# JoshuaLim007/VoxelEngine

Measured on AMD Instinct MI355X. Metric: Mrays/s primary+1-bounce @1080p, 8k×512×8k brickmap; % HBM roofline, higher is better.
Workload: dtype f32

## Files before the change

voxelengine_amd/csrc/vxrt_api.hip:

```cpp
#include "../../include/vxrt.h"
#include "vxrt_dist.hpp"
#include "vxrt_edit.hpp"
#include "vxrt_kernels.hpp"
#include "vxrt_islands.hpp"
#include "vxrt_nav.hpp"
#include "vxrt_region.hpp"
#include "vxrt_stream.hpp"

#include <algorithm>
#include <atomic>
#include <cmath>
#include <cstdio>
#include <cstdlib>
#include <cstring>
#include <initializer_list>
#include <map>
#include <new>
#include <set>
#include <string>
#include <utility>
#include <vector>

namespace vxrt {
hipError_t launch_render(const RenderArgs& A, bool stats, int variant, hipStream_t stream);
// ... 822 lines not shown
    VX_HIP(hipSetDevice(c->device));
    VX_HIP(hipDeviceSynchronize());
    unsigned long long now[vxrt::kStatCount] = {}, h[vxrt::kStatCount];
    std::vector<unsigned long long> rows((size_t)vxrt::kStatRows * vxrt::kStatRowStride);
    VX_HIP(hipMemcpy(rows.data(), c->d_stats, rows.size() * sizeof(unsigned long long), hipMemcpyDeviceToHost));
    for (unsigned r = 0; r < vxrt::kStatRows; ++r)
        for (int i = 0; i < vxrt::kStatCount; ++i)
            now[i] += rows[(size_t)r * vxrt::kStatRowStride + i];
    for (int i = 0; i < vxrt::kStatCount; ++i) {
        h[i] = now[i] - c->stats_base[i];
        c->stats_base[i] = now[i];
    }
    out->primary_rays = h[vxrt::kStatPrimary];
    out->shadow_rays = h[vxrt::kStatShadow];
    out->bounce_rays = h[vxrt::kStatBounce];
    out->primary_hits = h[vxrt::kStatPrimaryHits];
    out->coarse_probes = h[vxrt::kStatCoarseProbes];
    out->brick_entries = h[vxrt::kStatBrickEntries];
    out->fine_probes = h[vxrt::kStatFineProbes];
    out->dbg[0] = h[vxrt::kStatDbgIters];
    out->dbg[1] = h[vxrt::kStatDbgWalkLanes];
    out->dbg[2] = h[vxrt::kStatDbgEndRuns];
    out->dbg[3] = h[vxrt::kStatDbgBoxRuns];
    out->dbg[4] = h[vxrt::kStatDbgNextRuns];
    out->dbg[5] = h[vxrt::kStatDbgEndLanes];
    out->dbg[6] = h[vxrt::kStatDbgBoxLanes];
    out->dbg[7] = h[vxrt::kStatDbgNextLanes];
    out->dbg[8] = h[vxrt::kStatDbgLifetime];
    out->dbg[9] = h[vxrt::kStatDbgDrained];
    out->dbg[10] = h[vxrt::kStatDbgNextTicks];
    out->dbg[11] = h[vxrt::kStatDbgParkTicks];
    out->guard_slack_loads = h[vxrt::kStatGuardSlack];
    out->guard_stray_loads = h[vxrt::kStatGuardStray];
    return VXRT_OK;
}

int vxrt_deinterleave_strips(vxrt_ctx* c, uint32_t width, uint32_t height, int32_t strip_rows, int32_t strip_count,
                             const void* d_shards, uint64_t shard_stride_bytes, void* d_fb, void* stream)
{
    if (!c || !d_shards || !d_fb)
        return fail(VXRT_ERR_INVALID, "NULL argument");
    if (width % 4 != 0 || shard_stride_bytes % 16 != 0 || strip_rows <= 0 || strip_count <= 0)
        return fail(VXRT_ERR_INVALID, "width must be a multiple of 4 pixels and the shard stride of 16 bytes");
    VX_HIP(hipSetDevice(c->device));
    vxrt::launch_deinterleave(d_shards, shard_stride_bytes, d_fb, width, height, (uint32_t)strip_rows,
                              (uint32_t)strip_count, (hipStream_t)stream);
    VX_HIP(hipGetLastError());
    return VXRT_OK;
}

int vxrt_deinterleave_views(vxrt_ctx* c, uint32_t width, uint32_t height, int32_t strip_rows, int32_t strip_count,
                            const void* d_shards, uint64_t shard_stride_bytes, uint64_t view_stride_bytes, uint32_t n_views,
                            void* d_fb, uint64_t fb_stride_bytes, void* stream)
{
    if (!c || !d_shards || !d_fb)
        return fail(VXRT_ERR_INVALID, "NULL argument");
    if (width % 4 != 0 || shard_stride_bytes % 16 != 0 || view_stride_bytes % 16 != 0 || fb_stride_bytes % 16 != 0 ||
        strip_rows <= 0 || strip_count <= 0)
        return fail(VXRT_ERR_INVALID, "width must be a multiple of 4 pixels and the strides of 16 bytes");
    if (n_views > 65535u)
        return fail(VXRT_ERR_INVALID, "too many views");
    VX_HIP(hipSetDevice(c->device));
    vxrt::launch_deinterleave(d_shards, shard_stride_bytes, d_fb, width, height, (uint32_t)strip_rows, (uint32_t)strip_count,
                              (hipStream_t)stream, n_views, view_stride_bytes, fb_stride_bytes);
    VX_HIP(hipGetLastError());
    return VXRT_OK;
// ... 1198 lines not shown
```

voxelengine_amd/csrc/vxrt_batch_persist.hpp:

```cpp
#pragma once

#include "vxrt_kernels.hpp"
#include "vxrt_wave2.hpp"

namespace vxrt {

#ifndef VXRT_BATCH_VOTE_NEXT
#define VXRT_BATCH_VOTE_NEXT 2
#endif
#ifndef VXRT_BATCH_VOTE_END
#define VXRT_BATCH_VOTE_END 1
#endif
#ifndef VXRT_BATCH_VOTE_BOX
#define VXRT_BATCH_VOTE_BOX 2
#endif
#ifndef VXRT_BATCH_MASKED
#define VXRT_BATCH_MASKED 1
#endif
#ifndef VXRT_BATCH_PAIRS
#define VXRT_BATCH_PAIRS 1
#endif
constexpr uint32_t kBatchTicket = 64u;

#ifndef VXRT_BATCH_OCC
// ... 2 lines not shown
template <bool STATS, bool WIDE>
__global__ __launch_bounds__(64, VXRT_BATCH_OCC) void k_trace_batch_persist(BatchArgs B)
{
    __shared__ uint32_t cold_block[CF_TRACER_FIELDS * 64];
    const WorldView& W = B.W;
    const int lane = threadIdx.x & 63;
    constexpr unsigned long long kNone = ~0ull;

    WaveTracerT<WIDE> T;
    T.init(W, &cold_block[lane]);
    unsigned long long my_ray = kNone;
    unsigned long long chunk = 0;
    uint32_t used = kBatchTicket;
    const uint32_t tickets = (uint32_t)((B.n + kBatchTicket - 1u) / kBatchTicket);
    uint32_t queue_shard = blockIdx.x % kQueueShards;
    bool drained = false;
    uint32_t n_rays = 0, n_hits = 0;

    for (;;) {
        const unsigned long long m_walk = __ballot(T.st == ST_WALK);
        const unsigned long long m_box = __ballot(T.st == ST_BOX);
        const unsigned long long m_end = __ballot(waits_for_end(T.st));
        const unsigned long long m_next = __ballot(T.st == ST_DONE);
        if ((m_walk | m_box | m_end | m_next) == 0ull)
            break;
        int c_walk = __popcll(m_walk), c_box = __popcll(m_box), c_end = __popcll(m_end), c_next = __popcll(m_next);
        if (vote_run(c_box, c_walk, VXRT_BATCH_VOTE_BOX)) {
            T.template phase_box<STATS>(W);
            c_box = 0;
            c_walk = __popcll(__ballot(T.st == ST_WALK));
            c_end = __popcll(__ballot(waits_for_end(T.st)));
        }
        if (vote_run(c_end, c_walk + c_box, VXRT_BATCH_VOTE_END)) {
            T.template phase_end<STATS>(W);
            c_end = 0;
            c_walk = __popcll(__ballot(T.st == ST_WALK));
            c_next = __popcll(__ballot(T.st == ST_DONE));
        }
        if (vote_run(c_next, c_walk + c_box + c_end, VXRT_BATCH_VOTE_NEXT)) {
            bool c_hit = false;
            if (T.st == ST_DONE && my_ray != kNone) {
                TraceResult t;
                T.result(W, t);
                const unsigned long long i = my_ray;
                const f3 p = t.hit ? t.pos : mk3(kInf, kInf, kInf);
                B.pos[3 * i] = p.x;
                B.pos[3 * i + 1] = p.y;
                B.pos[3 * i + 2] = p.z;
                B.normal[3 * i] = t.normal.x;
                B.normal[3 * i + 1] = t.normal.y;
                B.normal[3 * i + 2] = t.normal.z;
                B.steps[i] = t.steps;
                if (B.hit)
                    B.hit[i] = t.hit ? 1 : 0;
                if (B.voxel)
                    B.voxel[i] = t.hit ? (long long)t.vx + (long long)W.X * ((long long)t.vy + (long long)W.Y * (long long)t.vz)
                                       : -1ll;
                c_hit = t.hit;
                my_ray = kNone;
            }
            bool got = false, launch = false;
            f3 o = mk3(0, 0, 0), d = mk3(1, 0, 0);
            unsigned long long want = __ballot(T.st == ST_DONE && my_ray == kNone);
            while (want != 0ull && !drained) {
                if (used >= kBatchTicket) {
                    const uint32_t t = queue_take(B.ticket, tickets, queue_shard, lane);
                    if (t == kQueueDry) {
// ... 9 lines not shown
                if (wants && rank < avail) {
                    const unsigned long long i = chunk + used + rank;
                    if (i < B.n) {
                        my_ray = i;
                        got = true;
                    }
                }
                const uint32_t asked = (uint32_t)__popcll(want);
                used += asked < avail ? asked : avail;
                want = __ballot(T.st == ST_DONE && my_ray == kNone);
            }
            if (got) {
                const unsigned long long j = my_ray;
                o = mk3(B.origins[3 * j], B.origins[3 * j + 1], B.origins[3 * j + 2]);
                d = mk3(B.dirs[3 * j], B.dirs[3 * j + 1], B.dirs[3 * j + 2]);
                if (ray_valid(o, d)) {
                    launch = true;
                } else {
                    B.pos[3 * j] = kInf;
                    B.pos[3 * j + 1] = kInf;
                    B.pos[3 * j + 2] = kInf;
                    B.normal[3 * j] = 0.0f;
                    B.normal[3 * j + 1] = 0.0f;
                    B.normal[3 * j + 2] = 0.0f;
                    B.steps[j] = 0;
                    if (B.hit)
                        B.hit[j] = 0;
                    if (B.voxel)
                        B.voxel[j] = -1ll;
                    my_ray = kNone;
                }
            }
            if (launch)
                T.begin_ray(W, o, d, B.max_steps);
            T.after_begin_ray(launch);
            if (drained && T.st == ST_DONE && my_ray == kNone)
                T.st = ST_IDLE;
            n_rays += (uint32_t)__popcll(__ballot(got));
            n_hits += (uint32_t)__popcll(__ballot(c_hit));
        }
        T.template probe_pairs<VXRT_BATCH_PAIRS, STATS, VXRT_BATCH_MASKED != 0>(W);
    }

    if (STATS && B.stats) {
        const unsigned long long p0 = wave_sum(T.cnt.coarse_probes), p1 = wave_sum(T.cnt.brick_entries),
                                 p2 = wave_sum(T.cnt.fine_probes), g0 = wave_sum(T.cnt.slack_loads), g1 = wave_sum(T.cnt.stray_loads);
        if (lane == 0) {
            unsigned long long* const stats = stats_row_of<kStatRows, kStatRowStride>(B.stats, blockIdx.x);
            atomicAdd(&stats[kStatGuardSlack], g0);
            atomicAdd(&stats[kStatGuardStray], g1);
            atomicAdd(&stats[kStatPrimary], (unsigned long long)n_rays);
            atomicAdd(&stats[kStatPrimaryHits], (unsigned long long)n_hits);
            atomicAdd(&stats[kStatCoarseProbes], p0);
            atomicAdd(&stats[kStatBrickEntries], p1);
            atomicAdd(&stats[kStatFineProbes], p2);
        }
    }
}

}
```

voxelengine_amd/csrc/vxrt_kernels.hpp:

```cpp
#pragma once

#include "vxrt_device.hpp"

namespace vxrt {

enum StatSlot {
    kStatPrimary = 0,
    kStatShadow,
    kStatBounce,
    kStatPrimaryHits,
    kStatCoarseProbes,
    kStatBrickEntries,
    kStatFineProbes,
    kStatDbgIters,
    kStatDbgWalkLanes,
    kStatDbgEndRuns,
    kStatDbgBoxRuns,
    kStatDbgNextRuns,
    kStatDbgEndLanes,
    kStatDbgBoxLanes,
    kStatDbgNextLanes,
    kStatDbgLifetime,
    kStatDbgDrained,
    kStatDbgNextTicks,
    kStatDbgParkTicks,
    kStatGuardSlack,
    kStatGuardStray,
    kStatCount
};

#ifndef VXRT_STAT_ROWS
#define VXRT_STAT_ROWS 64
#endif
constexpr unsigned kStatRows = VXRT_STAT_ROWS, kStatRowStride = 32;
static_assert(kStatCount <= (int)kStatRowStride, "a row holds every counter");

constexpr unsigned kMaxScheduledTileRows = 512;

struct RenderArgs {
    WorldView W;
    uint32_t width, height;
    uint32_t frame_number;
    uint32_t launch_rows;
    float kx, ky;
    float ortho_x, ortho_y, ratio;
    f3 origin, fwd, up, right;
    f3 light_dir, light_color, ambient;
    int mode, checkerboard, shadow, bounce_samples, bounce_all_hits, ortho;
    int bounce_depth;
    int strip_rows, strip_count, strip_index, compact;
    int strip_shift;
    uint8_t* fb;
    float* color_aov;
    long long* hit_aov;
    unsigned long long* stats;
    unsigned int* tile_counter;
    unsigned int persistent_waves;
    const unsigned int* tile_order;
    unsigned int row_order_n;
    uint16_t row_order[kMaxScheduledTileRows];
// ... 40 lines not shown
```

voxelengine_amd/csrc/vxrt_persist2.hpp:

```cpp
#pragma once

#include "vxrt_kernels.hpp"
#include "vxrt_wave2.hpp"

namespace vxrt {

enum : uint32_t { PX_NONE = 0u, PX_PRIMARY = 1u, PX_SHADOW = 2u, PX_BOUNCE = 3u, PX_BOUNCE2 = 4u };

struct PixelCoords {
    uint32_t tx, ty;
    int x, y;
    int out_row;
    bool live;
};

__device__ __forceinline__ PixelCoords pixel_coords(const RenderArgs& A, uint32_t frame_number, uint32_t tx, uint32_t row)
{
    PixelCoords c;
    c.tx = tx;
    c.ty = row;
    c.x = (int)tx;
    const bool sharded = A.strip_count > 1;
    if (sharded && !A.checkerboard) {
        const uint32_t sr = (uint32_t)A.strip_rows;
// ... 130 lines not shown
    __shared__ uint32_t cold_block[(CF_TRACER_FIELDS + PF_PIXEL_FIELDS) * 64 + 4];
    const WorldView& W = A_kern.W;
    const int lane = threadIdx.x & 63;
    uint32_t* const PX = &cold_block[CF_TRACER_FIELDS * 64 + lane];
    auto lane_view = [&](const RenderArgs& A, uint32_t v) -> LaneView {
        if (MULTI) {
            const ViewArgs& S = A.views[v];
            return LaneView{S.origin, S.fwd, S.up, S.right, S.frame_number, S.fb, S.color_aov, S.hit_aov};
        }
        return LaneView{A.origin, A.fwd, A.up, A.right, A.frame_number, A.fb, A.color_aov, A.hit_aov};
    };

    WaveTracerT<WIDE> T;
    T.init(W, &cold_block[lane]);
    uint32_t stage = PX_NONE;
    uint32_t px_tx = 0, px_row = 0;
    f3 position = mk3(0, 0, 0), color = mk3(0, 0, 0);
    uint32_t pcode = 0;
    int p_steps = 0;
    float occl = 0.0f;
    int sample = 0;
    uint32_t n_primary = 0, n_shadow = 0, n_bounce = 0, n_hits = 0;
    PX_ST_U(PF_STAGE, stage);
    if (lane < 4)
        cold_block[(CF_TRACER_FIELDS + PF_PIXEL_FIELDS) * 64 + lane] = 0u;

    uint32_t tile = 0, tile_used = 64u, tile_view = 0;
    uint32_t queue_shard = blockIdx.x % kQueueShards;
    bool drained = false;
    unsigned long long dg_iters = 0, dg_walk = 0, dg_drain = 0;
    unsigned int dg_runs[3] = {0, 0, 0}, dg_lanes[3] = {0, 0, 0};
    const unsigned long long dg_t0 = STATS ? wall_clock64() : 0ull;
    unsigned long long dg_next_ticks = 0, dg_park_ticks = 0;
#ifdef VXRT_TAIL_DEBUG
    unsigned long long px_t0 = 0;
#endif


    auto store_pixel = [&](const RenderArgs& A, const PixelCoords& pc, const LaneView& V, f3 origin, bool hit, f3 normal, f3 pos, f3 shaded) {
        PixelSink sink{A, pc.out_row, V.fb, V.color_aov};
        const int Wd = (int)A.width, Hd = (int)A.height;
        if (hit) {
            if (A.mode == 1) {
                f3 dv = pos - origin;
                float dist = sqrtf(dot3(dv, dv));
                const float wrap = (float)(1.0 + 1e-6);
                f3 hp = mk3(fmodf(pos.x / 128.0f, wrap), fmodf(pos.y / 128.0f, wrap), fmodf(pos.z / 128.0f, wrap));
                if (pc.x < (Wd >> 1) && pc.y < (Hd >> 1))
                    sink.put(pc.x, pc.y, normal);
                else if (pc.x >= (Wd >> 1) && pc.y < (Hd >> 1))
                    sink.put(pc.x, pc.y, hp);
                else if (pc.x < (Wd >> 1)) {
                } else
                    sink.put(pc.x, pc.y, mk3(dist * 0.01f, 0, 0));
            } else {
                if (!MULTI && A.accum)
                    shaded = accumulate_color(A, pc.out_row, pc.x, shaded);
                const float tx = shaded.x + 1.0f, ty = shaded.y + 1.0f, tz = shaded.z + 1.0f;
                f3 c = mk3(div_rn(shaded.x, tx, rcp_rn(tx)), div_rn(shaded.y, ty, rcp_rn(ty)), div_rn(shaded.z, tz, rcp_rn(tz)));
                const bool plain = !(((shaded.x == 0.0f) | ordinary(shaded.x)) & ((shaded.y == 0.0f) | ordinary(shaded.y)) &
                                     ((shaded.z == 0.0f) | ordinary(shaded.z)) & ordinary(tx) & ordinary(ty) & ordinary(tz));
                if (__ballot(plain) != 0ull)
                    c = mk3(shaded.x / (shaded.x + 1.0f), shaded.y / (shaded.y + 1.0f), shaded.z / (shaded.z + 1.0f));
                c = mk3(lo(hi(c.x, 0), 1), lo(hi(c.y, 0), 1), lo(hi(c.z, 0), 1));
                sink.put(pc.x, pc.y, c);
            }
        } else {
            sink.put(pc.x, pc.y, shaded);
        }
        if (pc.tx == (A.width >> 1) && pc.ty == (A.height >> 1)) {
            float ten = 10.0f;
            pin(ten);
            sink.put(pc.x, pc.y, mk3(ten, ten, ten));
        }
        if (A.mode == 1 && pc.x < (Wd >> 1) && pc.y > (Hd >> 1))
            sink.put(pc.x, pc.y, mk3((float)p_steps / 256.0f, 0, 0));
    };

    for (;;) {
        const unsigned long long m_walk = __ballot(T.st == ST_WALK);
        const unsigned long long m_box = __ballot(T.st == ST_BOX);
        const unsigned long long m_end = __ballot(waits_for_end(T.st));
        const unsigned long long m_next = __ballot(T.st == ST_DONE);
        if ((m_walk | m_box | m_end | m_next) == 0ull)
            break;
        const int n_walk = __popcll(m_walk), n_box = __popcll(m_box), n_end = __popcll(m_end), n_next = __popcll(m_next);
        if (STATS) {
            dg_iters += 1;
            dg_walk += (unsigned long long)n_walk;
            dg_drain += drained ? 1ull : 0ull;
        }

        int c_walk = n_walk, c_box = n_box, c_end = n_end, c_next = n_next;
        if (vote2(c_box, c_walk, VXRT_VOTE2_BOX, VXRT_VOTE2_ABS_BOX)) {
            if (STATS) {
                dg_runs[2] += 1u;
                dg_lanes[2] += (unsigned)c_box;
                dg_park_ticks -= wall_clock64();
            }
            T.template phase_box<STATS>(W);
            if (STATS)
                dg_park_ticks += wall_clock64();
            c_box = 0;
            c_walk = __popcll(__ballot(T.st == ST_WALK));
            c_end = __popcll(__ballot(waits_for_end(T.st)));
        }
        if (vote2(c_end, c_walk + c_box, VXRT_VOTE2_END, VXRT_VOTE2_ABS_END)) {
            if (STATS) {
                dg_runs[1] += 1u;
                dg_lanes[1] += (unsigned)c_end;
                dg_park_ticks -= wall_clock64();
            }
            T.template phase_end<STATS>(W);
            if (STATS)
                dg_park_ticks += wall_clock64();
            c_end = 0;
            c_walk = __popcll(__ballot(T.st == ST_WALK));
            c_next = __popcll(__ballot(T.st == ST_DONE));
        }
        if (vote2(c_next, c_walk + c_box + c_end, VXRT_VOTE2_NEXT, VXRT_VOTE2_ABS_NEXT)) {
            if (STATS) {
                dg_runs[0] += 1u;
                dg_lanes[0] += (unsigned)c_next;
                dg_next_ticks -= wall_clock64();
            }
            const RenderArgs& A = kernarg_reload(A_kern);
            const uint32_t ntx = (A.width + 7u) / 8u, nty = (A.launch_rows + 7u) / 8u, ntiles = ntx * nty;
            const f3 L = A.light_dir;
            const f3 sray = A.light_unit;
            PX_LD_U(PF_STAGE, stage);
            PX_LD_U(PF_TX, px_tx);
            PX_LD_U(PF_ROW, px_row);
            bool launch = false;
            bool c_hit = false, c_shadow = false, c_bounce = false;
            f3 l_origin = mk3(0, 0, 0), l_dir = mk3(1, 0, 0);
            int l_max = kMaxSteps;
            if (T.st == ST_DONE && stage != PX_NONE) {
                const LaneView V = lane_view(A, MULTI ? px_row >> 16 : 0u);
                const PixelCoords pc = pixel_coords(A, V.frame_number, px_tx, MULTI ? px_row & 0xFFFFu : px_row);
                const f3 origin = camera_origin(A, V, pc.x, pc.y);
                TraceResult r;
                T.result(W, r);
                bool finalize = false, do_shade = false, shadowed = false, bounce = false, bounce2 = false;
                if (stage == PX_PRIMARY) {
                    pcode = r.ncode;
                    p_steps = r.steps;
                    position = r.pos;
                    PX_ST_U(PF_PCODE, pcode);
                    PX_ST_U(PF_PSTEPS, p_steps);
                    PX_ST_POS();
// ... 55 lines not shown
                    } else {
                        finalize = true;
                    }
                } else if (stage == PX_BOUNCE || (BOUNCE2 && stage == PX_BOUNCE2)) {
                    PX_LD_F(PF_OCCL, occl);
                    PX_LD_I(PF_SAMPLE, sample);
                    if (!r.hit)
                        occl += stage == PX_BOUNCE ? 1.0f : 0.5f;
                    bounce2 = BOUNCE2 && stage == PX_BOUNCE && r.hit;
                    if (!bounce2) {
                        sample += 1;
                        if (sample < A.bounce_samples) {
                            bounce = true;
                        } else {
                            occl = div_rn(occl, A.bounce_samples_f, A.inv_bounce_samples);
                            PX_LD_COL();
                            color = color * occl;
                            PX_ST_COL();
                            stage = PX_PRIMARY;
                            finalize = true;
                        }
                    }
                    PX_ST_F(PF_OCCL, occl);
                    PX_ST_U(PF_SAMPLE, sample);
                }
                if (bounce || bounce2) {
                    PX_LD_POS();
                    const uint32_t seed = pc.ty * A.width + pc.tx;
                    const uint32_t si = seed + (uint32_t)sample * 1000u + (V.frame_number + 1u) * 1000u + (bounce2 ? 500u : 0u);
                    const f3 bn = mk3(bounce2 ? -r.normal.x : normal.x, bounce2 ? -r.normal.y : normal.y,
                                      bounce2 ? -r.normal.z : normal.z);
                    const f3 bo = mk3(bounce2 ? r.pos.x : position.x, bounce2 ? r.pos.y : position.y,
                                      bounce2 ? r.pos.z : position.z);
                    f3 sd = mk3(random_float(si) * 2 - 1, random_float(si * 10u) * 2 - 1, random_float(si * 100u) * 2 - 1);
                    {
                        const float sdd = dot3(sd, sd);
                        const f3 raw = sd;
                        sd = unit3_ordinary(raw, sdd);
                        if (__ballot(!ordinary(sdd)) != 0ull)
                            sd = unit3(raw);
                    }
                    if (dot3(sd, bn) < 0)
                        sd = reflect3(sd, bn);
                    c_bounce = true;
                    launch = true;
                    l_origin = bo + bn * 0.01f;
                    l_dir = sd;
                    l_max = 8;
                    stage = bounce2 ? PX_BOUNCE2 : PX_BOUNCE;
                }
                if (finalize) {
                    PX_LD_POS();
                    PX_LD_COL();
                    PX_LD_I(PF_PSTEPS, p_steps);
                    const LaneView Vs = lane_view(A, MULTI ? px_row >> 16 : 0u);
                    store_pixel(A, pc, Vs, origin, stage != PX_NONE, normal, position, color);
#ifdef VXRT_TAIL_DEBUG
                    if (STATS && V.color_aov) {
                        float* o = V.color_aov + ((size_t)pc.out_row * A.width + (size_t)pc.x) * 3;
                        o[0] = (float)(px_t0 & 0xFFFFFFull);
                        o[1] = (float)(wall_clock64() & 0xFFFFFFull);
                        o[2] = (float)p_steps;
                    }
#endif
                    stage = PX_NONE;
                }
            }
            bool got = false;
            unsigned long long want = __ballot(T.st == ST_DONE && stage == PX_NONE);
            while (want != 0ull && !drained) {
                if (tile_used >= 64u) {
                    tile = queue_take(A.tile_counter, ntiles * (MULTI ? A.nviews : 1u), VXRT_QUEUE_GRANULE, queue_shard, lane);
                    if (tile == kQueueDry) {
                        drained = true;
                        break;
                    }
                    tile_used = 0u;
                    if (MULTI) {
                        tile_view = tile / ntiles;
                        tile -= tile_view * ntiles;
                        const ViewArgs& S = A.views[tile_view];
                        if (S.row_order_n)
                            tile = (uint32_t)S.row_order[tile / ntx] * ntx + tile % ntx;
                    } else if (A.tile_order) {
                        tile = A.tile_order[tile];
                    } else if (A.row_order_n) {
                        tile = (uint32_t)A.row_order[tile / ntx] * ntx + tile % ntx;
                    }
                }
                const uint32_t avail = 64u - tile_used;
                const bool wants = ((want >> lane) & 1ull) != 0ull;
                const uint32_t rank = __builtin_amdgcn_mbcnt_hi((uint32_t)(want >> 32), __builtin_amdgcn_mbcnt_lo((uint32_t)want, 0u));
                if (wants && rank < avail) {
                    const uint32_t p = tile_used + rank;
                    px_tx = (tile % ntx) * 8u + (p & 7u);
                    px_row = (tile / ntx) * 8u + (p >> 3);
                    got = pixel_coords(A, MULTI ? A.views[tile_view].frame_number : A.frame_number, px_tx, px_row).live;
                    if (MULTI)
                        px_row |= tile_view << 16;
                }
                const uint32_t asked = (uint32_t)__popcll(want);
                tile_used += asked < avail ? asked : avail;
                want = __ballot(T.st == ST_DONE && stage == PX_NONE && !got);
            }
            if (got) {
                const LaneView V = lane_view(A, MULTI ? px_row >> 16 : 0u);
                const PixelCoords pc = pixel_coords(A, V.frame_number, px_tx, MULTI ? px_row & 0xFFFFu : px_row);
                camera_ray(A, V, pc.x, pc.y, l_origin, l_dir);
                color = l_dir;
                PX_ST_COL();
                l_max = kMaxSteps;
                launch = true;
                stage = PX_PRIMARY;
#ifdef VXRT_TAIL_DEBUG
                px_t0 = wall_clock64();
#endif
            }
            if (launch)
                T.begin_ray(W, l_origin, l_dir, l_max);
            T.after_begin_ray(launch);
            if (drained && T.st == ST_DONE && stage == PX_NONE)
                T.st = ST_IDLE;
            PX_ST_U(PF_STAGE, stage);
            PX_ST_U(PF_TX, px_tx);
            PX_ST_U(PF_ROW, px_row);
            {
                const uint32_t d0 = (uint32_t)__popcll(__ballot(got)), d1 = (uint32_t)__popcll(__ballot(c_shadow)),
                               d2 = (uint32_t)__popcll(__ballot(c_bounce)), d3 = (uint32_t)__popcll(__ballot(c_hit));
                if (lane == 0) {
                    uint32_t* const C = &cold_block[(CF_TRACER_FIELDS + PF_PIXEL_FIELDS) * 64];
                    C[0] += d0;
                    C[1] += d1;
                    C[2] += d2;
                    C[3] += d3;
                }
            }
            if (STATS)
                dg_next_ticks += wall_clock64();
        }

        T.template probe_pairs<VXRT_SUBROUNDS2, STATS>(W);
    }

    if (lane == 0) {
        const uint32_t* const C = &cold_block[(CF_TRACER_FIELDS + PF_PIXEL_FIELDS) * 64];
        n_primary = C[0];
        n_shadow = C[1];
        n_bounce = C[2];
        n_hits = C[3];
    }
    const unsigned long long s0 = n_primary, s1 = n_shadow, s2 = n_bounce, s3 = n_hits;
    unsigned long long* const stats = A_kern.stats ? stats_row_of<kStatRows, kStatRowStride>(A_kern.stats, blockIdx.x) : nullptr;
    if (lane == 0 && stats) {
        atomicAdd(&stats[kStatPrimary], s0);
        atomicAdd(&stats[kStatShadow], s1);
        atomicAdd(&stats[kStatBounce], s2);
        atomicAdd(&stats[kStatPrimaryHits], s3);
    }
    if (STATS) {
        const unsigned long long p0 = wave_sum(T.cnt.coarse_probes), p1 = wave_sum(T.cnt.brick_entries), p2 = wave_sum(T.cnt.fine_probes);
        const unsigned long long g0 = wave_sum(T.cnt.slack_loads), g1 = wave_sum(T.cnt.stray_loads);
        if (lane == 0 && stats) {
            atomicAdd(&stats[kStatCoarseProbes], p0);
            atomicAdd(&stats[kStatBrickEntries], p1);
            atomicAdd(&stats[kStatFineProbes], p2);
            atomicAdd(&stats[kStatGuardSlack], g0);
            atomicAdd(&stats[kStatGuardStray], g1);
            atomicAdd(&stats[kStatDbgIters], dg_iters);
            atomicAdd(&stats[kStatDbgWalkLanes], dg_walk);
            atomicAdd(&stats[kStatDbgNextRuns], (unsigned long long)dg_runs[0]);
            atomicAdd(&stats[kStatDbgEndRuns], (unsigned long long)dg_runs[1]);
            atomicAdd(&stats[kStatDbgBoxRuns], (unsigned long long)dg_runs[2]);
            atomicAdd(&stats[kStatDbgNextLanes], (unsigned long long)dg_lanes[0]);
            atomicAdd(&stats[kStatDbgEndLanes], (unsigned long long)dg_lanes[1]);
            atomicAdd(&stats[kStatDbgBoxLanes], (unsigned long long)dg_lanes[2]);
            atomicAdd(&stats[kStatDbgLifetime], wall_clock64() - dg_t0);
            atomicAdd(&stats[kStatDbgDrained], dg_drain);
            atomicAdd(&stats[kStatDbgNextTicks], dg_next_ticks);
            atomicAdd(&stats[kStatDbgParkTicks], dg_park_ticks);
        }
    }
}
#undef PX_LD_U
#undef PX_ST_U
#undef PX_LD_I
#undef PX_LD_F
#undef PX_ST_F
#undef PX_LD_POS
#undef PX_ST_POS
#undef PX_LD_COL
#undef PX_ST_COL

}
```

voxelengine_amd/csrc/vxrt_wave2.hpp:

```cpp
#pragma once

#include "vxrt_device.hpp"
#ifdef VXRT_HOST_DEBUG
#include <cstdio>
#include <cstdlib>
#endif

namespace vxrt {

enum : uint32_t { ST_WALK = 0u, ST_BOX = 1u, ST_END = 2u, ST_ENDHIT = 3u, ST_DONE = 4u, ST_IDLE = 5u };
__device__ __forceinline__ bool waits_for_end(uint32_t st) { return (st | 1u) == 3u; }
#ifndef VXRT_PROBE_GD
#define VXRT_PROBE_GD 0
#endif
#ifdef VXRT_HOST_CHECK
inline unsigned long long& host_unsuspected_exits() { static unsigned long long n = 0; return n; }
#endif

__device__ __forceinline__ f3 normal_decode(uint32_t c)
{
    float v = (c & 4u) ? -1.0f : 1.0f;
    uint32_t a = c & 3u;
    return mk3(a == 1u ? v : 0.0f, a == 2u ? v : 0.0f, a == 3u ? v : 0.0f);
}
// ... 36 lines not shown
{
    uint32_t r;
    asm("v_bfe_u32 %0, %1, %2, 1" : "=v"(r) : "v"(word), "v"(index));
    return r;
}
#else
__device__ __forceinline__ uint32_t bit_of(uint32_t word, uint32_t index) { return (word >> (index & 31u)) & 1u; }
#endif
__device__ __forceinline__ uint32_t rem_fx(uint32_t r) { return r & 0x7FFu; }
__device__ __forceinline__ uint32_t rem_fy(uint32_t r) { return (r >> 11) & 0x3FFu; }
__device__ __forceinline__ uint32_t rem_fz(uint32_t r) { return r >> 21; }
__device__ __forceinline__ uint32_t rem_sum(uint32_t r) { return rem_fx(r) + rem_fy(r) + rem_fz(r); }

template <bool WIDE>
struct WaveTracerT {
    f3 d;
    float ivx, ivy, ivz;
    float tn_x, tn_y, tn_z;
    uint32_t idx;
    uint32_t di_x, di_y, di_z;
    uint32_t rem, rp, rpp;
    float tl, tp;
    float t_hi;
    uint32_t fix;
    const uint32_t* bits;
    uint32_t st;
    f3 ws;
    uint32_t rem0;
    float t_hi_real;
    bool special;
    uint32_t dn;
    f3 point;
    lanemask_t fine_m;
    uint32_t* cold;
    RayCounters cnt;

    __device__ __forceinline__ bool lane_fine() const
    {
#ifdef VXRT_HOST_CHECK
        return (fine_m & 1ull) != 0ull;
#else
        return lane_test(fine_m);
#endif
    }

    __device__ __forceinline__ void init(const WorldView& W, uint32_t* cold_column)
    {
        cold = cold_column;
        st = ST_DONE;
        d = mk3(1.0f, 0.0f, 0.0f);
        ivx = ivy = ivz = 1.0f;
        tn_x = tn_y = tn_z = 0.0f;
        idx = (uint32_t)W.c_slice;
        di_x = di_y = di_z = 0u;
        rem = rp = rpp = 0u;
        tl = tp = 0.0f;
        t_hi = t_hi_real = kInf;
        special = false;
        dn = 6u;
        fix = 0u;
        bits = W.coarse_bits - (W.c_slice >> 5);
        ws = point = mk3(0, 0, 0);
        rem0 = 0u;
        fine_m = 0ull;
        cnt = RayCounters{0u, 0u, 0u, 0u, 0u};
    }

    __device__ __forceinline__ bool slab(f3 s, f3 bmin, f3 bmax, f3& p, uint32_t& code) const
    {
        float ax = (bmin.x - s.x) * ivx, bx = (bmax.x - s.x) * ivx;
        float ay = (bmin.y - s.y) * ivy, by = (bmax.y - s.y) * ivy;
        float az = (bmin.z - s.z) * ivz, bz = (bmax.z - s.z) * ivz;
        float nx = lo(ax, bx), fx = hi(ax, bx);
        float ny = lo(ay, by), fy = hi(ay, by);
        float nz = lo(az, bz), fz = hi(az, bz);
        float t_in = hi(hi(nx, ny), nz);
        float t_out = lo(lo(fx, fy), fz);
        p = mk3(s.x + t_in * d.x, s.y + t_in * d.y, s.z + t_in * d.z);
        code = (t_in == nx) ? (1u | (ivx < 0.0f ? 4u : 0u))
                            : (t_in == ny) ? (2u | (ivy < 0.0f ? 4u : 0u)) : (3u | (ivz < 0.0f ? 4u : 0u));
        return !(t_out < hi(t_in, 0.0f));
    }

    __device__ __forceinline__ bool slab_fast(f3 s, f3 bmin, f3 bmax, f3& p, uint32_t& code) const
    {
        float ax = (bmin.x - s.x) * ivx, bx = (bmax.x - s.x) * ivx;
        float ay = (bmin.y - s.y) * ivy, by = (bmax.y - s.y) * ivy;
        float az = (bmin.z - s.z) * ivz, bz = (bmax.z - s.z) * ivz;
        float nx = vmin(ax, bx), fx = vmax(ax, bx);
        float ny = vmin(ay, by), fy = vmax(ay, by);
        float nz = vmin(az, bz), fz = vmax(az, bz);
        float t_in = vmax3(nx, ny, nz);
        float t_out = vmin3(fx, fy, fz);
        p = mk3(s.x + t_in * d.x, s.y + t_in * d.y, s.z + t_in * d.z);
        const uint32_t c1 = ((__float_as_uint(ivx) >> 29) & 4u) | 1u, c2 = ((__float_as_uint(ivy) >> 29) & 4u) | 2u,
                       c3 = ((__float_as_uint(ivz) >> 29) & 4u) | 3u;
        const uint32_t c23 = t_in == ny ? c2 : c3;
// ... 65 lines not shown
        di_z = (row ^ nz) - nz;
        di_y = (slice ^ ny) - ny;
        const uint32_t ex = (uint32_t)(c_x - q_x), ey = (uint32_t)(c_y - q_y), ez = (uint32_t)(c_z - q_z);
        bool single = special;
        fix = 0u;
        if (__ballot(inside && (ex | ey | ez) != 0u) != 0ull) {
            const bool a0 = tn_x < tn_y && tn_x < tn_z;
            const bool a1 = !(tn_x < tn_y) && tn_y < tn_z;
            const bool a2 = !a0 && !a1;
            const uint32_t npend = ex + ey + ez;
            const bool simple = npend == 1u && ((ex != 0u && a0) || (ey != 0u && a1) || (ez != 0u && a2));
            fix = simple ? (((0u - ex) & di_x) | ((0u - ey) & di_y) | ((0u - ez) & di_z)) : 0u;
            single = single || (npend != 0u && !simple);
        }
        const uint32_t bxb = __float_as_uint(FINE ? W.ff : W.wmax_x), byb = __float_as_uint(FINE ? W.ff : W.wmax_y),
                       bzb = __float_as_uint(FINE ? W.ff : W.wmax_z);
        const float hx = (__uint_as_float(bxb & mx) - s.x) * ivx, hy = (__uint_as_float(byb & my) - s.y) * ivy,
                    hz = (__uint_as_float(bzb & mz) - s.z) * ivz;
        float hi_t = vmin3(hx, hy, hz);
        hi_t = hi_t - fabsf(hi_t) * (FINE ? kThrEpsFine : kThrEpsCoarse);
        hi_t = special ? -kInf : hi_t;
        if (FINE) {
            const uint32_t out = __float_as_uint(s.x) | __float_as_uint(s.y) | __float_as_uint(s.z) | __float_as_uint(W.ff - s.x) |
                                 __float_as_uint(W.ff - s.y) | __float_as_uint(W.ff - s.z);
            single = single || (int32_t)out < 0;
        }
        t_hi_real = hi_t;
        t_hi = single ? -kInf : hi_t;
        if (!FINE)
            bits = W.coarse_bits - (slice >> 5);
        st = inside ? (uint32_t)ST_WALK : (uint32_t)ST_END;
    }

    __device__ __forceinline__ void begin_ray(const WorldView& W, f3 origin, f3 ray, int max_steps_)
    {
        const float dd = dot3(ray, ray);
        d = unit3_ordinary(ray, dd);
        const float ex = d.x == 0 ? kFltEps : d.x, ey = d.y == 0 ? kFltEps : d.y, ez = d.z == 0 ? kFltEps : d.z;
        ivx = rcp_rn(ex);
        ivy = rcp_rn(ey);
        ivz = rcp_rn(ez);
        if (__ballot(!(ordinary(dd) & ordinary(ex) & ordinary(ey) & ordinary(ez))) != 0ull) {
            d = unit3(ray);
            ivx = 1.0f / (d.x == 0 ? kFltEps : d.x);
            ivy = 1.0f / (d.y == 0 ? kFltEps : d.y);
            ivz = 1.0f / (d.z == 0 ? kFltEps : d.z);
        }
        f3 s0 = mk3(origin.x * W.inv_f, origin.y * W.inv_f, origin.z * W.inv_f);
        uint32_t ec = 0u;
        if (!(s0.x >= 0 && s0.y >= 0 && s0.z >= 0 && s0.x < (float)W.cx && s0.y < (float)W.cy && s0.z < (float)W.cz)) {
            const float e = (float)1e-6;
            f3 p;
            uint32_t c;
            if (slab(s0, mk3(e, e, e), mk3(W.wmax_x, W.wmax_y, W.wmax_z), p, c)) {
                s0 = p;
                ec = c;
            }
        }
        cold[CF_RAY_CODES * 64] = ec | ((uint32_t)max_steps_ << 7);
        cold[CF_START_X * 64] = __float_as_uint(s0.x);
        cold[CF_START_Y * 64] = __float_as_uint(s0.y);
        cold[CF_START_Z * 64] = __float_as_uint(s0.z);
        cold[CF_LAST_CI * 64] = 0xFFFFFFFFu;
        cold[CF_TOTAL * 64] = 0u;
        special = !(fabsf(d.x) >= kMinFastDir && fabsf(d.y) >= kMinFastDir && fabsf(d.z) >= kMinFastDir) ||
                  __float_as_uint(s0.x) == 0x80000000u || __float_as_uint(s0.y) == 0x80000000u || __float_as_uint(s0.z) == 0x80000000u;
        dn = (d.x > 0 ? 0u : 1u) | (d.y > 0 ? 0u : 2u) | (d.z > 0 ? 0u : 4u);
        start_walk<false>(W, s0);
    }
    __device__ __forceinline__ void after_begin_ray(bool launched) { fine_m &= ~__ballot(launched); }

    __device__ __forceinline__ f3 cross_of(const WorldView& W, bool fine, uint32_t before, uint32_t dec, float t) const
    {
        int bx, by, bz;
        cells_of(W, fine, before, bx, by, bz);
        const bool on_x = dec == kRemDecX, on_y = dec == kRemDecY, on_z = dec == kRemDecZ;
        float face_x = (float)(bx + (d.x > 0 ? 1 : 0)), face_y = (float)(by + (d.y > 0 ? 1 : 0)), face_z = (float)(bz + (d.z > 0 ? 1 : 0));
        float lin_x = ws.x + (t * d.x), lin_y = ws.y + (t * d.y), lin_z = ws.z + (t * d.z);
        pin(face_x), pin(face_y), pin(face_z), pin(lin_x), pin(lin_y), pin(lin_z);
        return mk3(on_x ? face_x : lin_x, on_y ? face_y : lin_y, on_z ? face_z : lin_z);
    }

    __device__ __forceinline__ void walk_on(const WorldView& W, bool is_fine, bool lin_inside)
    {
        const bool single = t_hi == -kInf;
        if (__ballot(single) == 0ull)
            return;
        int x, y, z;
        cells_of(W, is_fine, rem, x, y, z);
        const int dmx = is_fine ? W.f : W.cx, dmy = is_fine ? W.f : W.cy, dmz = is_fine ? W.f : W.cz;
        const int row = is_fine ? W.f_row : W.c_row, slice = is_fine ? W.f_slice : W.c_slice;
        const uint32_t exact = cell_index(min(x, dmx - 1), min(y, dmy - 1), min(z, dmz - 1), row, dmz) + (uint32_t)slice;
        idx = single ? exact : idx;
        const bool pending = x == dmx || y == dmy || z == dmz;
        t_hi = (single && !pending && lin_inside) ? t_hi_real : t_hi;
    }

    template <bool STATS = false>
    __device__ __forceinline__ void phase_end(const WorldView& W)
    {
        const bool me = waits_for_end(st);
        const bool is_fine = lane_fine();
        bool go_coarse = false;
        if (me) {
            const bool hit = st == ST_ENDHIT;
            const uint32_t dec_last = rp - rem, dec_prev = rpp - rp;
            const bool stepped = dec_last != 0u;
            const bool guard = (rem & kRemGuards) != 0u;
            bool exiting = guard || !stepped;
            bool virt = false, exhausted = false;
            uint32_t offx = 0u, offy = 0u, offz = 0u;
            if (WIDE) {
                const uint32_t oxz = cold[CF_OFF_XZ * 64], oy = cold[CF_OFF_Y * 64];
                offx = oxz & 0xFFFFu;
                offy = oy;
                offz = oxz >> 16;
                const uint32_t off_k = dec_last == kRemDecX ? offx : (dec_last == kRemDecY ? offy : offz);
                virt = !is_fine && guard && stepped && off_k != 0u;
                exiting = exiting && !virt;
                exhausted = virt && !hit && rem0 - rem_sum(rp) + 1u >= (uint32_t)kMaxSteps;
            }
            const float F = W.ff;
            const f3 lin = mk3(ws.x + (tl * d.x), ws.y + (tl * d.y), ws.z + (tl * d.z));
            int bx, by, bz;
            cells_of(W, is_fine, rp, bx, by, bz);
            const f3 cr = mk3(dec_last == kRemDecX ? (float)(bx + (d.x > 0 ? 1 : 0)) : lin.x,
                              dec_last == kRemDecY ? (float)(by + (d.y > 0 ? 1 : 0)) : lin.y,
                              dec_last == kRemDecZ ? (float)(bz + (d.z > 0 ? 1 : 0)) : lin.z);
            float cr_lo = vmin3(cr.x, cr.y, cr.z), cr_hi = vmax3(cr.x, cr.y, cr.z);
            float lin_lo = vmin3(lin.x, lin.y, lin.z), lin_hi = vmax3(lin.x, lin.y, lin.z);
            f3 pc_prev = cross_of(W, is_fine, rpp, dec_prev, tp);
            pin(cr_lo), pin(cr_hi), pin(lin_lo), pin(lin_hi);
// ... 59 lines not shown
                        float ux = ulp_fast(sx, d.x), uy = ulp_fast(sy, d.y), uz = ulp_fast(sz, d.z);
                        const uint32_t m_or = (__float_as_uint(sx) & 0x7FFFFFFFu) - 1u | (__float_as_uint(sy) & 0x7FFFFFFFu) - 1u |
                                              (__float_as_uint(sz) & 0x7FFFFFFFu) - 1u;
                        if (__ballot(m_or >= 0x7F7FFFFFu || special) != 0ull) {
                            ux = ulp_step(sx, d.x < 0);
                            uy = ulp_step(sy, d.y < 0);
                            uz = ulp_step(sz, d.z < 0);
                        }
                        sx = nudge ? ux : sx;
                        sy = nudge ? uy : sy;
                        sz = nudge ? uz : sz;
                        const bool snap = nudge & trunc_equals(sx, fx) & trunc_equals(sy, fy) & trunc_equals(sz, fz);
                        if (snap) {
                            const int nca = (int)(cold[CF_BOX_CODES * 64] >> 3);
                            const int axis = nca & 3;
                            const int ncx = hx + ((nca >> 2) & 1) + (axis == 0 ? (d.x > 0 ? 1 : -1) : 0);
                            const int ncy = hy + ((nca >> 3) & 1) + (axis == 1 ? (d.y > 0 ? 1 : -1) : 0);
                            const int ncz = hz + ((nca >> 4) & 1) + (axis == 2 ? (d.z > 0 ? 1 : -1) : 0);
                            const float gx = (float)ncx - sx, gy = (float)ncy - sy, gz = (float)ncz - sz;
                            const float mx = fabsf(gx), my = fabsf(gy), mz = fabsf(gz);
                            const bool snap_x = (mx < my) & (mx < mz);
                            const bool snap_y = !snap_x & (my < mx) & (my < mz);
                            const bool snap_z = !snap_x & !snap_y;
                            sx = snap_x ? sx + gx : sx;
                            sy = snap_y ? sy + gy : sy;
                            sz = snap_z ? sz + gz : sz;
                        }
                    }
                    cold[CF_START_X * 64] = __float_as_uint(sx);
                    cold[CF_START_Y * 64] = __float_as_uint(sy);
                    cold[CF_START_Z * 64] = __float_as_uint(sz);
                    const bool restart = total_ < (int)(cold[CF_RAY_CODES * 64] >> 7);
                    if (restart) {
                        start_walk<false>(W, mk3(sx, sy, sz));
                        go_coarse = true;
                    } else {
                        st = ST_DONE;
                    }
                }
            }
        }
        fine_m &= ~__ballot(go_coarse);
    }

    template <bool STATS = false>
    __device__ __forceinline__ void phase_box(const WorldView& W)
    {
        bool go_fine = false;
        if (st == ST_BOX) {
            int x, y, z;
            cells_of(W, false, rp, x, y, z);
            const int qx = min(x, W.cx - 1), qy = min(y, W.cy - 1), qz = min(z, W.cz - 1);
            const uint32_t ci = cell_index(qx, qy, qz, W.c_row, W.cz);
            const uint2 meta = W.cell_meta[ci];
            const uint32_t e = meta.y;
            const float fqx = (float)qx, fqy = (float)qy, fqz = (float)qz;
            f3 bmin = mk3(((float)(e & 31u) + 0) * W.inv_f + fqx, ((float)((e >> 5) & 31u) + 0) * W.inv_f + fqy,
                          ((float)((e >> 10) & 31u) + 0) * W.inv_f + fqz);
            f3 bmax = mk3(((float)((e >> 15) & 31u) + 1) * W.inv_f + fqx, ((float)((e >> 20) & 31u) + 1) * W.inv_f + fqy,
                          ((float)((e >> 25) & 31u) + 1) * W.inv_f + fqz);
            f3 bp;
            uint32_t bc;
            bool box_hit = slab_fast(ws, bmin, bmax, bp, bc) && bmin.x <= bmax.x;
            if (__ballot(special) != 0ull) {
                if (special)
                    box_hit = slab(ws, bmin, bmax, bp, bc) && bmin.x <= bmax.x;
            }
            if (box_hit) {
                const uint32_t steps = rem0 - rem_sum(rp);
                cold[CF_TOTAL * 64] += steps;
                if (STATS)
                    cnt.coarse_probes += steps + 1u;
                point.x = steps != 0u ? bp.x : ws.x;
                point.y = steps != 0u ? bp.y : ws.y;
                point.z = steps != 0u ? bp.z : ws.z;
// ... 186 lines not shown
    __device__ __forceinline__ void result(const WorldView& W, TraceResult& out) const
    {
        const uint32_t ray_codes = cold[CF_RAY_CODES * 64];
        const bool hit = (ray_codes & 0x40u) != 0u;
        const int total_ = (int)cold[CF_TOTAL * 64];
        const int hx = (int)cold[CF_CHX * 64], hy = (int)cold[CF_CHY * 64], hz = (int)cold[CF_CHZ * 64];
        out.hit = hit;
        out.steps = total_;
        const bool is_fine = lane_fine();
        const float ox = (float)hx * W.ff, oy = (float)hy * W.ff, oz = (float)hz * W.ff;
        out.pos = mk3(is_fine ? point.x + ox : point.x * W.ff, is_fine ? point.y + oy : point.y * W.ff,
                      is_fine ? point.z + oz : point.z * W.ff);
        int x, y, z;
        cells_of(W, true, rp, x, y, z);
        out.vx = hx * W.f + min(x, W.f - 1);
        out.vy = hy * W.f + min(y, W.f - 1);
        out.vz = hz * W.f + min(z, W.f - 1);
        const bool at_entry = hit && total_ == 0;
        out.ncode = at_entry ? (ray_codes & 7u) : ((ray_codes >> 3) & 7u);
        out.normal = normal_decode(out.ncode);
        if (at_entry)
            out.pos = mk3(__uint_as_float(cold[CF_START_X * 64]) * W.ff, __uint_as_float(cold[CF_START_Y * 64]) * W.ff,
                          __uint_as_float(cold[CF_START_Z * 64]) * W.ff);
    }
};

template <int PAIRS = 1, bool STATS = false, bool WIDE = false, bool MASKED = false>
__device__ inline void trace_wave2(const WorldView& W, const int max_steps, const bool active, const f3 origin, const f3 ray,
                                   TraceResult& out, uint32_t* cold_column, RayCounters* counters = nullptr)
{
    WaveTracerT<WIDE> T;
    T.init(W, cold_column);
    if (active)
        T.begin_ray(W, origin, ray, max_steps);
    T.after_begin_ray(active);
    for (;;) {
        const unsigned long long m_walk = __ballot(T.st == ST_WALK);
        const unsigned long long m_box = __ballot(T.st == ST_BOX);
        const unsigned long long m_end = __ballot(waits_for_end(T.st));
        if ((m_walk | m_box | m_end) == 0ull)
            break;
        const int n_walk = __popcll(m_walk), n_box = __popcll(m_box), n_end = __popcll(m_end);
        if (vote_run(n_end, n_walk + n_box, VXRT_VOTE_END))
            T.template phase_end<STATS>(W);
        if (vote_run(n_box, n_walk, VXRT_VOTE_BOX))
            T.template phase_box<STATS>(W);
        T.template probe_pairs<PAIRS, STATS, MASKED>(W);
    }
    if (active)
        T.result(W, out);
    if (STATS && counters) {
        counters->coarse_probes += T.cnt.coarse_probes;
        counters->brick_entries += T.cnt.brick_entries;
        counters->fine_probes += T.cnt.fine_probes;
        counters->slack_loads += T.cnt.slack_loads;
        counters->stray_loads += T.cnt.stray_loads;
    }
}

}
```

Before: 8534.

## Defer walk starts so ray-finish and end-phase restarts share one start_walk

Ray begin and end-of-walk restarts no longer call start_walk inline. They now set ST_WALK and mark the lane in a pending mask, and a single start_pending call runs start_walk once per round for all marked lanes. This merges two divergent executions of the same expensive code into one per wavefront round. It also moves the pixel tx/row stores into the branch that assigns a new pixel, pins a constant in the bounce sampler, and adds debug counters for how often both paths fire in the same round. The risk is that some lanes sit briefly in a half-initialised walk state between phases.

```diff
diff --git a/voxelengine_amd/csrc/vxrt_api.hip b/voxelengine_amd/csrc/vxrt_api.hip
--- a/voxelengine_amd/csrc/vxrt_api.hip
+++ b/voxelengine_amd/csrc/vxrt_api.hip
@@ -878,6 +878,11 @@
     out->dbg[11] = h[vxrt::kStatDbgParkTicks];
     out->guard_slack_loads = h[vxrt::kStatGuardSlack];
     out->guard_stray_loads = h[vxrt::kStatGuardStray];
+#ifdef VXRT_EXPERIMENTS
+    if (getenv("VXRT_PRINT_COSTART"))
+        fprintf(stderr, "vxrt: rounds with the end-of-walk and the ray-finished phase %llu, with walk starts from both %llu, of %llu rounds\n",
+                h[vxrt::kStatDbgCoRuns], h[vxrt::kStatDbgCoStarts], h[vxrt::kStatDbgIters]);
+#endif
     return VXRT_OK;
 }
 
diff --git a/voxelengine_amd/csrc/vxrt_batch_persist.hpp b/voxelengine_amd/csrc/vxrt_batch_persist.hpp
--- a/voxelengine_amd/csrc/vxrt_batch_persist.hpp
+++ b/voxelengine_amd/csrc/vxrt_batch_persist.hpp
@@ -58,7 +58,7 @@
             c_end = __popcll(__ballot(waits_for_end(T.st)));
         }
         if (vote_run(c_end, c_walk + c_box, VXRT_BATCH_VOTE_END)) {
-            T.template phase_end<STATS>(W);
+            T.template phase_end_deferred<STATS>(W);
             c_end = 0;
             c_walk = __popcll(__ballot(T.st == ST_WALK));
             c_next = __popcll(__ballot(T.st == ST_DONE));
@@ -134,13 +134,14 @@
                 }
             }
             if (launch)
-                T.begin_ray(W, o, d, B.max_steps);
-            T.after_begin_ray(launch);
+                T.begin_ray_deferred(W, o, d, B.max_steps);
+            T.after_begin_ray_deferred(launch);
             if (drained && T.st == ST_DONE && my_ray == kNone)
                 T.st = ST_IDLE;
             n_rays += (uint32_t)__popcll(__ballot(got));
             n_hits += (uint32_t)__popcll(__ballot(c_hit));
         }
+        T.start_pending(W);
         T.template probe_pairs<VXRT_BATCH_PAIRS, STATS, VXRT_BATCH_MASKED != 0>(W);
     }
 
diff --git a/voxelengine_amd/csrc/vxrt_kernels.hpp b/voxelengine_amd/csrc/vxrt_kernels.hpp
--- a/voxelengine_amd/csrc/vxrt_kernels.hpp
+++ b/voxelengine_amd/csrc/vxrt_kernels.hpp
@@ -26,6 +26,8 @@
     kStatDbgParkTicks,
     kStatGuardSlack,
     kStatGuardStray,
+    kStatDbgCoRuns,
+    kStatDbgCoStarts,
     kStatCount
 };
 
diff --git a/voxelengine_amd/csrc/vxrt_persist2.hpp b/voxelengine_amd/csrc/vxrt_persist2.hpp
--- a/voxelengine_amd/csrc/vxrt_persist2.hpp
+++ b/voxelengine_amd/csrc/vxrt_persist2.hpp
@@ -186,6 +186,7 @@
     unsigned int dg_runs[3] = {0, 0, 0}, dg_lanes[3] = {0, 0, 0};
     const unsigned long long dg_t0 = STATS ? wall_clock64() : 0ull;
     unsigned long long dg_next_ticks = 0, dg_park_ticks = 0;
+    unsigned long long dg_co_runs = 0, dg_co_starts = 0;
 #ifdef VXRT_TAIL_DEBUG
     unsigned long long px_t0 = 0;
 #endif
@@ -246,6 +247,7 @@
         }
 
         int c_walk = n_walk, c_box = n_box, c_end = n_end, c_next = n_next;
+        bool dg_end_ran = false, dg_end_restarted = false;
         if (vote2(c_box, c_walk, VXRT_VOTE2_BOX, VXRT_VOTE2_ABS_BOX)) {
             if (STATS) {
                 dg_runs[2] += 1u;
@@ -265,11 +267,15 @@
                 dg_lanes[1] += (unsigned)c_end;
                 dg_park_ticks -= wall_clock64();
             }
-            T.template phase_end<STATS>(W);
+            T.template phase_end_deferred<STATS>(W);
             if (STATS)
                 dg_park_ticks += wall_clock64();
             c_end = 0;
             c_walk = __popcll(__ballot(T.st == ST_WALK));
+            if (STATS) {
+                dg_end_ran = true;
+                dg_end_restarted = T.pend_m != 0ull;
+            }
             c_next = __popcll(__ballot(T.st == ST_DONE));
         }
         if (vote2(c_next, c_walk + c_box + c_end, VXRT_VOTE2_NEXT, VXRT_VOTE2_ABS_NEXT)) {
@@ -391,7 +397,9 @@
                                       bounce2 ? -r.normal.z : normal.z);
                     const f3 bo = mk3(bounce2 ? r.pos.x : position.x, bounce2 ? r.pos.y : position.y,
                                       bounce2 ? r.pos.z : position.z);
-                    f3 sd = mk3(random_float(si) * 2 - 1, random_float(si * 10u) * 2 - 1, random_float(si * 100u) * 2 - 1);
+                    float two = 2.0f;
+                    pin(two);
+                    f3 sd = mk3(random_float(si) * two - 1, random_float(si * 10u) * two - 1, random_float(si * 100u) * two - 1);
                     {
                         const float sdd = dot3(sd, sd);
                         const f3 raw = sd;
@@ -426,6 +434,7 @@
                 }
             }
             bool got = false;
+            uint32_t new_tx = 0, new_row = 0;
             unsigned long long want = __ballot(T.st == ST_DONE && stage == PX_NONE);
             while (want != 0ull && !drained) {
                 if (tile_used >= 64u) {
@@ -452,19 +461,21 @@
                 const uint32_t rank = __builtin_amdgcn_mbcnt_hi((uint32_t)(want >> 32), __builtin_amdgcn_mbcnt_lo((uint32_t)want, 0u));
                 if (wants && rank < avail) {
                     const uint32_t p = tile_used + rank;
-                    px_tx = (tile % ntx) * 8u + (p & 7u);
-                    px_row = (tile / ntx) * 8u + (p >> 3);
-                    got = pixel_coords(A, MULTI ? A.views[tile_view].frame_number : A.frame_number, px_tx, px_row).live;
+                    new_tx = (tile % ntx) * 8u + (p & 7u);
+                    new_row = (tile / ntx) * 8u + (p >> 3);
+                    got = pixel_coords(A, MULTI ? A.views[tile_view].frame_number : A.frame_number, new_tx, new_row).live;
                     if (MULTI)
-                        px_row |= tile_view << 16;
+                        new_row |= tile_view << 16;
                 }
                 const uint32_t asked = (uint32_t)__popcll(want);
                 tile_used += asked < avail ? asked : avail;
                 want = __ballot(T.st == ST_DONE && stage == PX_NONE && !got);
             }
             if (got) {
-                const LaneView V = lane_view(A, MULTI ? px_row >> 16 : 0u);
-                const PixelCoords pc = pixel_coords(A, V.frame_number, px_tx, MULTI ? px_row & 0xFFFFu : px_row);
+                PX_ST_U(PF_TX, new_tx);
+                PX_ST_U(PF_ROW, new_row);
+                const LaneView V = lane_view(A, MULTI ? new_row >> 16 : 0u);
+                const PixelCoords pc = pixel_coords(A, V.frame_number, new_tx, MULTI ? new_row & 0xFFFFu : new_row);
                 camera_ray(A, V, pc.x, pc.y, l_origin, l_dir);
                 color = l_dir;
                 PX_ST_COL();
@@ -476,13 +487,15 @@
 #endif
             }
             if (launch)
-                T.begin_ray(W, l_origin, l_dir, l_max);
-            T.after_begin_ray(launch);
+                T.begin_ray_deferred(W, l_origin, l_dir, l_max);
+            T.after_begin_ray_deferred(launch);
+            if (STATS) {
+                dg_co_runs += dg_end_ran ? 1ull : 0ull;
+                dg_co_starts += (dg_end_restarted && __ballot(launch) != 0ull) ? 1ull : 0ull;
+            }
             if (drained && T.st == ST_DONE && stage == PX_NONE)
                 T.st = ST_IDLE;
             PX_ST_U(PF_STAGE, stage);
-            PX_ST_U(PF_TX, px_tx);
-            PX_ST_U(PF_ROW, px_row);
             {
                 const uint32_t d0 = (uint32_t)__popcll(__ballot(got)), d1 = (uint32_t)__popcll(__ballot(c_shadow)),
                                d2 = (uint32_t)__popcll(__ballot(c_bounce)), d3 = (uint32_t)__popcll(__ballot(c_hit));
@@ -498,6 +511,7 @@
                 dg_next_ticks += wall_clock64();
         }
 
+        T.start_pending(W);
         T.template probe_pairs<VXRT_SUBROUNDS2, STATS>(W);
     }
 
@@ -537,6 +551,8 @@
             atomicAdd(&stats[kStatDbgDrained], dg_drain);
             atomicAdd(&stats[kStatDbgNextTicks], dg_next_ticks);
             atomicAdd(&stats[kStatDbgParkTicks], dg_park_ticks);
+            atomicAdd(&stats[kStatDbgCoRuns], dg_co_runs);
+            atomicAdd(&stats[kStatDbgCoStarts], dg_co_starts);
         }
     }
 }
diff --git a/voxelengine_amd/csrc/vxrt_wave2.hpp b/voxelengine_amd/csrc/vxrt_wave2.hpp
--- a/voxelengine_amd/csrc/vxrt_wave2.hpp
+++ b/voxelengine_amd/csrc/vxrt_wave2.hpp
@@ -92,9 +92,18 @@
     uint32_t dn;
     f3 point;
     lanemask_t fine_m;
+    lanemask_t pend_m;
     uint32_t* cold;
     RayCounters cnt;
 
+    __device__ __forceinline__ bool lane_pending() const
+    {
+#ifdef VXRT_HOST_CHECK
+        return (pend_m & 1ull) != 0ull;
+#else
+        return lane_test(pend_m);
+#endif
+    }
     __device__ __forceinline__ bool lane_fine() const
     {
 #ifdef VXRT_HOST_CHECK
@@ -123,6 +132,7 @@
         ws = point = mk3(0, 0, 0);
         rem0 = 0u;
         fine_m = 0ull;
+        pend_m = 0ull;
         cnt = RayCounters{0u, 0u, 0u, 0u, 0u};
     }
 
@@ -254,7 +264,23 @@
         st = inside ? (uint32_t)ST_WALK : (uint32_t)ST_END;
     }
 
+    __device__ __forceinline__ void start_pending(const WorldView& W)
+    {
+        if (pend_m == 0ull)
+            return;
+        if (lane_pending())
+            start_walk<false>(W, mk3(__uint_as_float(cold[CF_START_X * 64]), __uint_as_float(cold[CF_START_Y * 64]),
+                                     __uint_as_float(cold[CF_START_Z * 64])));
+        pend_m = 0ull;
+    }
+
     __device__ __forceinline__ void begin_ray(const WorldView& W, f3 origin, f3 ray, int max_steps_)
+    {
+        begin_ray_deferred(W, origin, ray, max_steps_);
+        start_walk<false>(W, mk3(__uint_as_float(cold[CF_START_X * 64]), __uint_as_float(cold[CF_START_Y * 64]),
+                                 __uint_as_float(cold[CF_START_Z * 64])));
+    }
+    __device__ __forceinline__ void begin_ray_deferred(const WorldView& W, f3 origin, f3 ray, int max_steps_)
     {
         const float dd = dot3(ray, ray);
         d = unit3_ordinary(ray, dd);
@@ -288,9 +314,15 @@
         special = !(fabsf(d.x) >= kMinFastDir && fabsf(d.y) >= kMinFastDir && fabsf(d.z) >= kMinFastDir) ||
                   __float_as_uint(s0.x) == 0x80000000u || __float_as_uint(s0.y) == 0x80000000u || __float_as_uint(s0.z) == 0x80000000u;
         dn = (d.x > 0 ? 0u : 1u) | (d.y > 0 ? 0u : 2u) | (d.z > 0 ? 0u : 4u);
-        start_walk<false>(W, s0);
+        st = ST_WALK;
     }
     __device__ __forceinline__ void after_begin_ray(bool launched) { fine_m &= ~__ballot(launched); }
+    __device__ __forceinline__ void after_begin_ray_deferred(bool launched)
+    {
+        const lanemask_t m = __ballot(launched);
+        fine_m &= ~m;
+        pend_m |= m;
+    }
 
     __device__ __forceinline__ f3 cross_of(const WorldView& W, bool fine, uint32_t before, uint32_t dec, float t) const
     {
@@ -320,6 +352,12 @@
 
     template <bool STATS = false>
     __device__ __forceinline__ void phase_end(const WorldView& W)
+    {
+        phase_end_deferred<STATS>(W);
+        start_pending(W);
+    }
+    template <bool STATS = false>
+    __device__ __forceinline__ void phase_end_deferred(const WorldView& W)
     {
         const bool me = waits_for_end(st);
         const bool is_fine = lane_fine();
@@ -445,7 +483,7 @@
                     cold[CF_START_Z * 64] = __float_as_uint(sz);
                     const bool restart = total_ < (int)(cold[CF_RAY_CODES * 64] >> 7);
                     if (restart) {
-                        start_walk<false>(W, mk3(sx, sy, sz));
+                        st = ST_WALK;
                         go_coarse = true;
                     } else {
                         st = ST_DONE;
@@ -453,7 +491,9 @@
                 }
             }
         }
-        fine_m &= ~__ballot(go_coarse);
+        const lanemask_t m = __ballot(go_coarse);
+        fine_m &= ~m;
+        pend_m |= m;
     }
 
     template <bool STATS = false>
@@ -706,8 +746,8 @@
     WaveTracerT<WIDE> T;
     T.init(W, cold_column);
     if (active)
-        T.begin_ray(W, origin, ray, max_steps);
-    T.after_begin_ray(active);
+        T.begin_ray_deferred(W, origin, ray, max_steps);
+    T.after_begin_ray_deferred(active);
     for (;;) {
         const unsigned long long m_walk = __ballot(T.st == ST_WALK);
         const unsigned long long m_box = __ballot(T.st == ST_BOX);
@@ -716,9 +756,10 @@
             break;
         const int n_walk = __popcll(m_walk), n_box = __popcll(m_box), n_end = __popcll(m_end);
         if (vote_run(n_end, n_walk + n_box, VXRT_VOTE_END))
-            T.template phase_end<STATS>(W);
+            T.template phase_end_deferred<STATS>(W);
         if (vote_run(n_box, n_walk, VXRT_VOTE_BOX))
             T.template phase_box<STATS>(W);
+        T.start_pending(W);
         T.template probe_pairs<PAIRS, STATS, MASKED>(W);
     }
     if (active)
```

After: 8648 (median of 6 runs). 1.01x the previous value.
